# simplew4y/VeritasFi

Measured on AMD Instinct MI355X. Metric: queries/sec top-100 over 10Mx768 corpus, higher is better.
Workload: dtype f16

## Files before the change

veritasfi_amd/build.py:

```python
from __future__ import annotations

import os
import shutil
import subprocess
import sys

HERE = os.path.dirname(os.path.abspath(__file__))
CSRC = os.path.join(HERE, "csrc")
LIBDIR = os.path.join(HERE, "lib")
LIB = os.path.join(LIBDIR, os.environ.get("VF_BUILD_LIB", "libveritasfi_hip.so"))
SOURCES = ["vf_kernels.hip", "vf_api.hip", "vf_transformer.hip", "vf_sparse.hip"]
HEADERS = ["vf_internal.h", os.path.join("..", "..", "include", "veritasfi_hip.h"), "vf_ksplit_geom.h"]
ARCH = "gfx950"
FLAGS = ["-O3", "-std=c++17", "-fPIC", f"--offload-arch={ARCH}", "-Wall", "-Wno-unused-function"]
EXTRA = os.environ.get("VF_BUILD_FLAGS", "").split()


def _hipcc() -> str:
    for cand in (shutil.which("hipcc"), "/opt/rocm/bin/hipcc"):
        if cand and os.path.exists(cand):
            return cand
    raise RuntimeError("hipcc not found: the HIP library cannot be built (no fallback exists)")


def _stale(target: str, deps) -> bool:
    if not os.path.exists(target):
        return True
    t = os.path.getmtime(target)
    return any(os.path.exists(d) and os.path.getmtime(d) > t for d in deps)


KEPT_HOOKS = ("vf_debug_force_no_peer", "vf_debug_small_allocs")
TEST_LIB = os.path.join(LIBDIR, "libvf_test.so")


# ... 63 lines not shown
```

veritasfi_amd/csrc/vf_api.hip:

```cpp
#include "../../include/veritasfi_hip.h"
#include "vf_internal.h"

#include <fcntl.h>
#include <float.h>
#include <sys/stat.h>
#include <unistd.h>
#include <math.h>
#include <string.h>

#include <algorithm>
#include <atomic>
#include <mutex>
#include <string>
#include <vector>

using namespace vf;

static thread_local std::string g_err;

static int fail(int code, const std::string& msg) {
    g_err = msg;
    return code;
}
int vf::set_error(int code, const std::string& msg) { return fail(code, msg); }
// ... 181 lines not shown
            ix->rows_scan = ix->rows_orig;
            ix->owns_scan = false;
        } else {
            VF_HIP(hipMalloc((void**)&ix->rows_scan, (size_t)ix->n * ix->dp * scan_esz));
            ix->owns_scan = true;
            scan_out = ix->rows_scan;
        }
    }
    VF_HIP(launch_prep_rows(ix->rows_orig, dt, ix->n, ix->d, ix->dp, scan_out, ix->norm, ix->inv_scan, nullptr));
    VF_TRY(build_image(ix, ix->scan_image));
    if (ix->n > 0 && ix->n <= kSmallN) {
        VF_HIP(hipMalloc((void**)&ix->cn_cache, (size_t)ix->n * ix->d * sizeof(float)));
        VF_HIP(launch_normalize_rows(ix->rows_orig, dt, 0, ix->n, ix->d, ix->norm, ix->cn_cache, nullptr));
    }
    VF_HIP(hipDeviceSynchronize());
    return VF_OK;
}

constexpr int64_t kSplitMaxRows = 6'000'000;
constexpr int64_t kScan2rMinRows = 1'100'000;
static bool scan2r_auto_width(int dp, bool f8) { return f8 ? (dp == 768 || dp == 1024) : (dp == 768 || dp == 1024 || dp == 512 || dp == 384); }
static int64_t split_limit(const vf_index* ix) {
    const bool r_rows = ix->dtype != VF_DTYPE_FP8_E4M3 && ix->scan_impl != 4 && ix->scan_impl != 1 && ix->scan_impl != 3 && !ix->steal_opt &&
                        scan2r_auto_width(ix->dp, false) && scan2r_stage_cap(ix->dp, kMaxBatch, 0) >= 256;
    return r_rows ? INT64_MAX : kSplitMaxRows;
}
static int64_t resolved_aux(const vf_index* ix) {
    if (ix->aux_applied >= 0) return ix->aux_applied;
    int64_t a = ix->aux_cus >= 0 ? ix->aux_cus : (ix->n <= split_limit(ix) ? 32 : 0);
    if (a <= 0 || ix->n_cu < 64 || a * 2 > ix->n_cu) return 0;
    return a;
}
static bool resolved_overlap(const vf_index* ix) {
    return ix->overlap_scans >= 0 ? ix->overlap_scans != 0 : resolved_aux(ix) > 0;
}

constexpr int kImageMaxK = 128;
constexpr int64_t kImageMinRows = 4'000'000;
constexpr double kImageMaxRho = 1.0 / 64;
constexpr size_t kImageHeadroom = (size_t)8 << 30;
constexpr int kImageMfmaAuto = 1;
static bool image_eligible(const vf_index* ix) {
    return ix->shards.empty() && (ix->dtype == VF_DTYPE_F16 || ix->dtype == VF_DTYPE_F32) && ix->n >= kImageMinRows &&
           ix->n < (int64_t)0xFFFFFFFFll && ix->dp == 768 && scan2r_stage_cap(ix->dp, kMaxBatch, 2) >= 256;
}
static float* image_offsets(const vf_index* ix) { return ix->inv_img ? ix->inv_img + ix->n + 64 : nullptr; }
static void free_image(vf_index* ix) {
    if (ix->rows_img) (void)hipFree(ix->rows_img);
    if (ix->inv_img) (void)hipFree(ix->inv_img);
    ix->rows_img = nullptr; ix->inv_img = nullptr; ix->rho_max = ix->rho_mean = 0.0f;
}
static int build_image(vf_index* ix, int64_t mode) {
    if (mode == 0 || ix->rows_img || !image_eligible(ix)) return VF_OK;
    const size_t bytes = (size_t)ix->n * ix->dp, ibytes = 2 * ((size_t)ix->n + 64) * sizeof(float);
    if (mode == 1) {
        size_t free_b = 0, total_b = 0;
        if (hipMemGetInfo(&free_b, &total_b) != hipSuccess) { (void)hipGetLastError(); return VF_OK; }
        if (free_b < bytes + ibytes + kImageHeadroom) return VF_OK;
    }
    if (hipMalloc((void**)&ix->rows_img, bytes) != hipSuccess || hipMalloc((void**)&ix->inv_img, ibytes) != hipSuccess) {
        (void)hipGetLastError();
        free_image(ix);
        return mode == 2 ? fail(VF_ENOMEM, "scan_image = 2: the int8 row image does not fit in device memory") : VF_OK;
    }
    u32* d_rho = nullptr;
    VF_HIP(hipMalloc((void**)&d_rho, 2 * sizeof(u32)));
    VF_HIP(hipMemset(d_rho, 0, 2 * sizeof(u32)));
// ... 458 lines not shown
    *tau_band = (int)ceil(band * (kHistBins / 2)) + 1;
    *fine_band = (int)ceil(band * (kHistBins / 2) * 16) + 1;
}

extern "C" int vf_debug_image_bound(int32_t d, int32_t dtype, float rho_mean, float* eps, int32_t* tau_band, int32_t* fine_band) {
    if (!eps || !tau_band || !fine_band || d <= 0) return fail(VF_EINVAL, "vf_debug_image_bound: bad argument");
    int tb = 0, fb = 0;
    image_bound(d, dtype, rho_mean, eps, &tb, &fb);
    *tau_band = tb; *fine_band = fb;
    return VF_OK;
}

extern "C" int vf_debug_image_q8_bound(float rho_q, float eps_img, int32_t tau_band, int32_t fine_band, float* eps_q, int32_t* tau_band_q,
                                       int32_t* fine_band_q) {
    if (!eps_q || !tau_band_q || !fine_band_q) return fail(VF_EINVAL, "vf_debug_image_q8_bound: bad argument");
    const Q8Bound b = image_q8_bound(rho_q);
    *eps_q = image_q8_eps(eps_img, b.eps_add);
    *tau_band_q = tau_band + b.tau_bins; *fine_band_q = fine_band + b.fine_bins;
    return VF_OK;
}

static int image_planes(const vf_index* ix, int qt) {
    const int m = ix->image_mfma < 0 ? kImageMfmaAuto : (int)ix->image_mfma;
    return (m >= 1 && scan2r_stage_cap(ix->dp, qt, 2 + m) >= 256) ? m : 0;
}

static bool image_serves(const vf_index* ix, int k, int qt) {
    return ix->rows_img && k <= kImageMaxK && (ix->scan_impl == 2 || ix->scan_impl == 5) && !ix->steal_opt && ix->sample_impl != 0 &&
           scan2r_stage_cap(ix->dp, qt, 2) >= 256;
}

static FusedPlan make_plan(const vf_index* ix, int k, bool image = false) {
    FusedPlan p;
    p.image = image; p.tau_band = 0; p.fine_band = 0;
    int margin = ix->margin >= 0 ? (int)ix->margin : std::max(24, k / 4);
    const double u16 = 1.0 / 2048.0;
    const float eps_plan = (float)(u16 * (ix->dtype == VF_DTYPE_F32 ? 2.0 : 1.0) + sqrt((double)ix->d) * ldexp(1.0, -24) +
                                   2.0 * ix->d * ldexp(1.0, -24) + 1e-6);
    if (ix->margin < 0 && ksplit_width(ix)) {
        const double z = sqrt(2.0 * log(std::max(3.0, (double)ix->n / k)));
        margin = std::max(margin, (int)ceil(2.5 * eps_plan * k * z * sqrt((double)ix->d)));
    }
    p.kprime = ix->margin >= 0 ? k + margin : (k + margin + 31) / 32 * 32;
    p.kprime = std::min(p.kprime, 4096);
    int cap = kMaxCap;
    while (cap < 4 * p.kprime && cap < 16384) cap <<= 1;
    if (ix->cap_opt > 0) { cap = 1; while (cap < ix->cap_opt) cap <<= 1; cap = std::min(cap, 16384); }
    while (cap < 2 * p.kprime) cap <<= 1;
    p.cap = cap;
    const int64_t scan_cus = ix->n_cu - resolved_aux(ix);
    int64_t wgs = std::min<int64_t>(scan_cus, std::max<int64_t>(1, ix->n / 512));
    if (ix->waves_opt > 0) wgs = std::max<int64_t>(1, ix->waves_opt / (kScanThreads / 64));
// ... 206 lines not shown
            VF_TRY(s.qimg8.ensure((size_t)ix->dp * kMaxBatch * 2));
            VF_TRY(s.epsq.ensure(kMaxBatch * sizeof(float)));
            VF_TRY(s.qscale.ensure(kMaxBatch * sizeof(float)));
            VF_TRY(s.bandq.ensure(2 * kMaxBatch * sizeof(int)));
            VF_HIP(launch_prep_q8(qn_b, nb, ix->d, ix->dp, qt, s.image_i8, (signed char*)s.qimg8.p, s.qscale.as<float>(), s.epsq.as<float>(), s.bandq.as<int>(),
                                  p.eps, p.tau_band, p.fine_band, st));
            a.qimg = (const _Float16*)s.qimg8.p; a.q_scale = s.qscale.as<float>(); a.band_q = s.bandq.as<int>();
        }
        a.n = ix->n; a.dp = ix->dp; a.row_bytes = (long long)ix->dp * (ix->dtype == VF_DTYPE_FP8_E4M3 ? 1 : 2); a.total_waves = p.total_waves; a.samp = p.samp;
        if (p.image) { a.rows = (const char*)ix->rows_img; a.inv_scan = ix->inv_img; a.off_scan = image_offsets(ix); a.row_bytes = ix->dp; }
        a.s0 = s.s0.as<float>(); a.wg_base = s.wgbase.as<long long>(); a.cnt = s.cnt.as<u32>(); a.tau_bin = s.tau.as<int>(); a.hist = s.hist.as<u32>();
        a.cand = s.cand.as<u64>(); a.cap = p.cap; a.kprime = p.kprime; a.tau_band = p.tau_band;
        a.hist_coarse = s.hist_coarse.as<u32>(); a.stage_cap = ks ? scan_ksplit_stage_cap(ix->dp) : scan_stage_cap(ix->dp, qt);
        a.tile_cnt = ix->steal_opt ? s.tilecnt.as<u32>() : nullptr; a.scan_grid = p.grid;
        a.dbg = nullptr;
        if (ix->debug & 128) { VF_TRY(s.dbg.ensure((size_t)p.total_waves * ((ix->debug & 512) ? 72 : 4) * sizeof(u64))); a.dbg = s.dbg.as<u64>(); if (ix->debug & 512) VF_HIP(hipMemsetAsync(s.dbg.p, 0, s.dbg.bytes, st)); }
        a.refresh_every = (int)std::min<int64_t>(256, std::max<int64_t>(4, std::max<int64_t>(1, ix->refresh_every) * nb / kMaxBatch));
        while (a.refresh_every & (a.refresh_every - 1)) a.refresh_every &= a.refresh_every - 1;
        a.nq = nb; a.debug = (int)ix->debug;
        if (ix->n / p.total_waves < p.samp)
            VF_HIP(hipMemsetAsync(a.s0, 0xFF, (size_t)qt * p.total_waves * p.samp * sizeof(float), st));
        const bool f8rows = ix->dtype == VF_DTYPE_FP8_E4M3 || p.image;
        const bool r_f8_auto = f8rows && ix->scan_impl == 2 && ix->n > kScan2rMinRows && !ix->steal_opt && scan2r_auto_width(ix->dp, true);
        const bool sample_r = p.image || (ix->sample_impl != 0 && ix->scan_impl != 1 && scan2r_stage_cap(ix->dp, qt, f8rows) >= 256 &&
                              (ix->sample_impl == 1 || (!f8rows && s.scan_stream != s.stream && scan2r_auto_width(ix->dp, false)) || r_f8_auto));
        if (ks) {
            VF_HIP(launch_scan_ksplit(a, kModeSample, p.grid, st));
        } else if (sample_r) {
            const int64_t sg_r = ix->sample_grid > 0 ? ix->sample_grid : (s.scan_stream != s.stream ? resolved_aux(ix) : p.grid);
            ScanArgs as = a;
            as.stage_cap = 0;
            VF_HIP(launch_scan2r_sample(as, qt, (int)std::min<int64_t>(std::max<int64_t>(sg_r, 1), p.grid), p.image ? img_f8 : (int)f8rows, st));
        } else {
        const int64_t sg_opt = ix->sample_grid >= 0 ? ix->sample_grid : (s.scan_stream != s.stream ? 4 * resolved_aux(ix) : 0);
        const int sgrid = sg_opt > 0 ? (int)std::min<int64_t>(sg_opt, p.grid) : p.grid;
        VF_HIP(launch_scan(a, kModeSample, qt, sgrid, (int)ix->scan_g, ix->dtype == VF_DTYPE_FP8_E4M3, st));
        }
        VF_HIP(launch_sel0(a, qt, st));
        hipStream_t sst = s.scan_stream;
        if (sst != st) {
            VF_HIP(hipEventRecord(s.ev_pro, st));
            VF_HIP(hipStreamWaitEvent(sst, s.ev_pro, 0));
        }
        if (!resolved_overlap(ix))
            for (int o = 0; o < kSlots; ++o)
                if (o != slot_id && ix->slots[o].ev_scan) VF_HIP(hipStreamWaitEvent(sst, ix->slots[o].ev_scan, 0));
        if (s.timed && b0 == 0) {
// ... 2 lines not shown
                VF_HIP(hipEventRecord(ix->ev_span, sst));
                ix->span_started = true;
            }
            ix->span_slot[slot_id] = true;
            VF_HIP(hipEventRecord(s.ev_t[0], sst));
        }
        const int f8 = ix->dtype == VF_DTYPE_FP8_E4M3 ? 1 : 0;
        const int cap2 = ((ix->scan_impl == 3 || ((ix->scan_impl == 2 || ix->scan_impl == 4 || ix->scan_impl == 5) && !f8)) && !ix->steal_opt) ? scan2_stage_cap(ix->dp, qt, f8) : 0;
        const bool r_auto = ix->scan_impl == 2 && ix->n > kScan2rMinRows && scan2r_auto_width(ix->dp, f8 != 0) && (f8 || (s.scan_stream != s.stream && resolved_overlap(ix)));
#ifdef VF_EXPERIMENTS
        const bool dbg_r = f8 || !(ix->debug & (32 | 64));
#else
        const bool dbg_r = true;
#endif
        const int capr = ((ix->scan_impl == 5 || r_auto) && !ix->steal_opt && dbg_r) ? scan2r_stage_cap(ix->dp, qt, f8) : 0;
        if (ks) {
            VF_HIP(launch_scan_ksplit(a, kModeMain, p.grid, sst));
            s.scan_kernel = 6;
        } else if (p.image) {
            ScanArgs a2 = a;
            a2.stage_cap = scan2r_stage_cap(ix->dp, qt, img_f8);
            VF_HIP(launch_scan2r(a2, qt, p.grid, img_f8, sst));
            s.scan_kernel = 5;
        } else if (capr >= 256) {
            ScanArgs a2 = a;
            a2.stage_cap = capr;
            VF_HIP(launch_scan2r(a2, qt, p.grid, f8, sst));
            s.scan_kernel = 5;
        } else if (cap2 >= 256) {
            ScanArgs a2 = a;
            a2.stage_cap = cap2;
#ifdef VF_EXPERIMENTS
            if (ix->debug & 32) {
                const bool fresh = s.sib.bytes < 4096;
                VF_TRY(s.sib.ensure(4096));
                if (fresh) VF_HIP(hipMemsetAsync(s.sib.p, 0xFF, 4096, st));
                a2.sib = s.sib.as<u32>();
            }
#endif
            VF_HIP(launch_scan2(a2, qt, p.grid, f8, sst));
            s.scan_kernel = 2;
        } else {
            VF_HIP(launch_scan(a, kModeMain, qt, p.grid, (int)ix->scan_g, ix->dtype == VF_DTYPE_FP8_E4M3, sst));
            s.scan_kernel = 1;
        }
        VF_HIP(hipEventRecord(s.ev_scan, sst));
        if (s.timed && b0 == 0) {
// ... 729 lines not shown
```

veritasfi_amd/csrc/vf_internal.h:

```cpp
#pragma once
#include <hip/hip_runtime.h>
#include <math.h>
#include <stdint.h>

#include "../../include/veritasfi_hip.h"

#include <string>

#include "vf_ksplit_geom.h"

namespace vf {

int set_error(int code, const std::string& msg);

typedef unsigned long long u64;
typedef unsigned int u32;

struct DeviceGuard {
    int prev = -1;
    DeviceGuard() { if (hipGetDevice(&prev) != hipSuccess) prev = -1; }
    ~DeviceGuard() { if (prev >= 0) (void)hipSetDevice(prev); }
    DeviceGuard(const DeviceGuard&) = delete;
    DeviceGuard& operator=(const DeviceGuard&) = delete;
};

__device__ __forceinline__ u32 orderkey(float f) {
    f = f + 0.0f;
    const u32 b = __float_as_uint(f);
    return b ^ ((b >> 31) ? 0xFFFFFFFFu : 0x80000000u);
}
__device__ __forceinline__ float unorderkey(u32 k) {
    return __uint_as_float((k & 0x80000000u) ? (k ^ 0x80000000u) : ~k);
// ... 98 lines not shown
hipError_t launch_prep_rows(const void* rows, int dt , long long n, int d, int dp,
                            void* scan ,
                            float* norm, float* inv_scan, hipStream_t s);
hipError_t launch_prep_image(const void* rows, int dt, long long n, int d, int dp, const float* norm, unsigned char* img,
                             float* inv_img, float* off_img, u32* rho_max_bits, float* rho_sum, hipStream_t s);
hipError_t launch_prep_queries(const float* q, int nq, int d, int dp, int qn_tile ,
                               float* qn, _Float16* qimg, hipStream_t s);
hipError_t launch_normalize_rows(const void* rows, int dt , long long row0, long long nrows, int d,
                                 const float* norm, float* out, hipStream_t s);
hipError_t launch_normalize_rows_gather(const void* rows, int dt, const long long* sel , int nsel, int d,
                                        const float* norm, float* out, hipStream_t s);
hipError_t launch_dense_dot16(const float* qn, int nq, const float* cn, long long nrows, int d,
                              float* out, long long out_stride, hipStream_t s);
hipError_t launch_sort_rows(const float* scores, long long score_stride, int nq, int n, int k,
                            long long id_base, long long* out_ids, float* out_scores, int out_stride,
                            hipStream_t s);
hipError_t launch_scan(const ScanArgs& a, int mode, int qn_tile, int grid, int want_g ,
                       int rows_are_fp8, hipStream_t s);
hipError_t launch_debug_cvt_e4m3(const unsigned char* in, float* out, int count, hipStream_t s);
hipError_t launch_debug_mfma_i8(const signed char* A, const signed char* B, int* C, hipStream_t s);
hipError_t launch_scan2(const ScanArgs& a, int qn_tile, int grid, int rows_are_fp8, hipStream_t s);
size_t scan2_lds_bytes(int dp, int qn_tile, int stage_cap);
int scan2_stage_cap(int dp, int qn_tile, int rows_are_fp8);
size_t scan2r_lds_bytes(int dp, int qn_tile, int stage_cap, int f8);
int scan2r_stage_cap(int dp, int qn_tile, int f8);
hipError_t launch_scan2r(const ScanArgs& a, int qn_tile, int grid, int f8, hipStream_t s);
hipError_t launch_scan2r_sample(const ScanArgs& a, int qn_tile, int grid, int f8, hipStream_t s);
hipError_t launch_scan_ksplit(const ScanArgs& a, int mode, int grid, hipStream_t s);
size_t scan_ksplit_lds_bytes(int dp, int stage_cap);
int scan_ksplit_stage_cap(int dp);
hipError_t launch_scan_wide(const ScanArgs& a, int mode, int rows_are_fp8, hipStream_t s);
size_t scan_wide_lds_bytes(int stage_cap);
hipError_t launch_prep_wide8(const float* qn, int nq, int d, int dp, int qtot, unsigned char* img8, float* eps_q, hipStream_t s);
hipError_t launch_scan_wide8(const ScanArgs& a, int waves , hipStream_t s);
int scan_wide8_stage_cap(int waves);
int scan_wide8_occupancy(int waves, int stage_cap);
hipError_t launch_prep_q8(const float* qn, int nq, int d, int dp, int qn_tile, int planes , signed char* img8, float* q_scale, float* eps_q, int* band_q,
                          float eps_img, int tau_band, int fine_band, hipStream_t s);
hipError_t launch_sel0(const ScanArgs& a, int qn_tile, hipStream_t s);
hipError_t launch_final(FinalArgs a, int nq, hipStream_t s);
hipError_t launch_merge_topk(const long long* ids_parts, const float* score_parts, int nparts, int nq,
                             int k, long long* ids, float* scores, hipStream_t s);
hipError_t launch_merge_topk_packed(const void* parts, int nparts, int nq, int k, long long* ids, float* scores,
                                    hipStream_t s);
hipError_t launch_fuse_rank(const float* a, const float* b, int n, float* out, long long* order,
                            hipStream_t s);
// ... 7 lines not shown
```

veritasfi_amd/csrc/vf_kernels.hip:

```cpp
#include "vf_internal.h"

#include <float.h>
#include <algorithm>
#include <type_traits>

#include <mutex>

namespace vf {

typedef _Float16 h8 __attribute__((ext_vector_type(8)));
typedef _Float16 h4 __attribute__((ext_vector_type(4)));
typedef float f16v __attribute__((ext_vector_type(16)));
typedef int i4v __attribute__((ext_vector_type(4)));
typedef int i16v __attribute__((ext_vector_type(16)));
typedef int i8v __attribute__((ext_vector_type(8)));

__device__ __forceinline__ float group16_tree(float acc) {
    acc = acc + __shfl_down(acc, 8, 16);
    acc = acc + __shfl_down(acc, 4, 16);
    acc = acc + __shfl_down(acc, 2, 16);
    acc = acc + __shfl_down(acc, 1, 16);
    return acc;
}

// ... 727 lines not shown
                 __builtin_amdgcn_readlane((int)v, 32) | __builtin_amdgcn_readlane((int)v, 48));
}
__device__ __forceinline__ u32 wave_sum_u32(u32 v) {
    v += VF_DPP_ROR(v, 1);
    v += VF_DPP_ROR(v, 2);
    v += VF_DPP_ROR(v, 4);
    v += VF_DPP_ROR(v, 8);
    return (u32)(__builtin_amdgcn_readlane((int)v, 0) + __builtin_amdgcn_readlane((int)v, 16) +
                 __builtin_amdgcn_readlane((int)v, 32) + __builtin_amdgcn_readlane((int)v, 48));
}

template <int NT, int MODE>
__device__ __forceinline__ void epi_prefetch(EpiRegs<NT>& e, const ScanArgs& a, long long t0, int lane, bool sync_tau) {
    e.inv_lane = a.inv_scan[t0 + (lane & 31)];
    e.sync_tau = sync_tau;
    if (MODE == kModeMain && sync_tau) {
#pragma unroll
        for (int nt = 0; nt < NT; ++nt)
            e.tau_g[nt] = __hip_atomic_load(a.tau_bin + nt * kQueryTile + (lane & 31), __ATOMIC_RELAXED,
                                            __HIP_MEMORY_SCOPE_AGENT);
    }
}

template <int NT, int MODE, bool PUBLISH = true, bool INV_LDS = false, bool OFF = false>
__device__ __forceinline__ void tile_epilogue(const ScanArgs& a, const f16v (&acc)[NT], const EpiRegs<NT>& e,
                                              long long t0, long long hi, long long s0_slot, int lane, char* ctl) {
    const int r31 = lane & 31, h = lane >> 5;
    auto inv_of = [&](int reg) {
        const int r0 = (reg & 3) + 8 * (reg >> 2);
        const float lo_half = __builtin_bit_cast(float, __builtin_amdgcn_readlane(__builtin_bit_cast(int, e.inv_lane), r0));
        const float hi_half = __builtin_bit_cast(float, __builtin_amdgcn_readlane(__builtin_bit_cast(int, e.inv_lane), r0 + 4));
        return h ? hi_half : lo_half;
    };
    auto off_of = [&](int reg) {
        const int r0 = (reg & 3) + 8 * (reg >> 2);
        const float lo_half = __builtin_bit_cast(float, __builtin_amdgcn_readlane(__builtin_bit_cast(int, e.off_lane), r0));
        const float hi_half = __builtin_bit_cast(float, __builtin_amdgcn_readlane(__builtin_bit_cast(int, e.off_lane), r0 + 4));
        return h ? hi_half : lo_half;
    };
    if (MODE == kModeSample) {
        const long long s0_stride = (long long)a.total_waves * a.samp;
#pragma unroll
        for (int nt = 0; nt < NT; ++nt) {
            const int q = nt * kQueryTile + r31;
#pragma unroll
            for (int reg = 0; reg < 16; ++reg) {
                const int rr = (reg & 3) + 8 * (reg >> 2) + 4 * h;
                if constexpr (OFF) {
                    if (t0 + rr < hi) a.s0[(long long)q * s0_stride + s0_slot + rr] = acc[nt][reg] * inv_of(reg) + off_of(reg);
// ... 53 lines not shown
        }
        any |= bin_x(top) >= tb[nt];
    }
    if (__ballot(any) == 0ull) return;
    u32 mask = 0;
#pragma unroll
    for (int nt = 0; nt < NT; ++nt)
#pragma unroll
        for (int reg = 0; reg < 16; ++reg) mask |= (bin_x(m[nt * 16 + reg]) >= tb[nt]) ? (1u << (nt * 16 + reg)) : 0u;
    const unsigned long long hot = __ballot(mask != 0u);
    if (hot == 0ull) return;
    if (a.debug & 4) return;
    u32 umask = 0u, total = 0u;
    if (__popcll(hot) <= 8) {
        for (unsigned long long hb = hot; hb != 0ull; hb &= hb - 1ull) {
            const u32 m = (u32)__builtin_amdgcn_readlane((int)mask, __builtin_ctzll(hb));
            umask |= m;
            total += (u32)__popc(m);
        }
    } else {
        umask = wave_or_u32(mask);
        total = wave_sum_u32((u32)__popc(mask));
    }
    u32* stage_cnt = (u32*)ctl;
    uint4* stage_ent = (uint4*)(ctl + kCtlBytes);
    const u32 rs = 31u - (u32)__builtin_clz((u32)a.refresh_every | 1u);
    const u32 R = 1u << rs;
    u32 base = 0;
    if (lane == 0) base = atomicAdd(stage_cnt, total);
    base = (u32)__builtin_amdgcn_readfirstlane((int)base);
    const bool need = (base >> rs) != ((base + total) >> rs);
    if (a.debug & 8) return;
    u32 run = base;
    const u32 edge = (((base + total) >> rs) << rs) - 1u;
    int qq = 0;
    for (u32 um = umask; um != 0u; um &= um - 1u) {
        const int pair = __builtin_ctz(um);
        const int nt = pair >> 4, reg = pair & 15;
        const int q = nt * kQueryTile + r31;
        const bool mine = ((mask >> pair) & 1u) != 0u;
        const unsigned long long bal = __ballot(mine);
        if (mine) {
            const u32 slot = run + __builtin_amdgcn_mbcnt_hi((u32)(bal >> 32), __builtin_amdgcn_mbcnt_lo((u32)bal, 0u));
            const int rr = (reg & 3) + 8 * (reg >> 2) + 4 * h;
            const float sc = m[pair];
            const u32 bin = (u32)bin_of_x(bin_x(sc));
            const u32 key = orderkey(sc), row = (u32)(t0 + rr);
            if (slot < (u32)a.stage_cap) {
                stage_ent[slot] = make_uint4(row, key, (u32)q | (bin << 8), 1u);
            } else {
                const u32 gs = atomicAdd(a.cnt + q * kCntStride, 1u);
                if (gs < (u32)a.cap) a.cand[(long long)q * a.cap + gs] = ((u64)key << 32) | (u64)row;
                atomicAdd(a.hist + (long long)q * kHistBins + bin, 1u);
                atomicAdd(a.hist_coarse + q * 64 + (bin >> 5), 1u);
            }
        }
        const u32 nxt = run + (u32)__popcll(bal);
        if (run <= edge && edge < nxt) qq = nt * kQueryTile + ((__ffsll((long long)bal) - 1) & 31);
        run = nxt;
    }
    if (a.debug & 2) return;
    if constexpr (!PUBLISH) return;
    if (need) {
        const int nb = wave_tau_two_level(a.hist_coarse + qq * 64, a.hist + (long long)qq * kHistBins, a.kprime, lane) - (a.band_q ? a.band_q[qq] : a.tau_band);
        if (lane == 0 && nb > 0) {
            atomicMax(a.tau_bin + qq, nb);
            atomicMax(tau_lds + qq, nb);
        }
        for (u32 blk = base >> rs; blk < (base + total) >> rs; ++blk)
        for (u32 j = (u32)lane; j < R; j += 64u) {
            const u32 idx = (blk << rs) + j;
            if (idx >= (u32)a.stage_cap) break;
            const uint4 en = stage_ent[idx];
            if (en.w == 1u) {
                const u32 q = en.z & 0xFFu, bin = en.z >> 8;
                if (q < (u32)QN_of<NT>() && bin < (u32)kHistBins) {
                    atomicAdd(a.hist + (long long)q * kHistBins + bin, 1u);
                    atomicAdd(a.hist_coarse + q * 64 + (bin >> 5), 1u);
                }
            }
        }
    }
}

#define VF_ISSUE(BUF, ...)                                                        \
    do {                                                                          \
        if constexpr (F8 != 0) issue_loads_f8<G>(BUF, __VA_ARGS__);               \
        else issue_loads<G>(BUF, __VA_ARGS__);                                    \
    } while (0)
#define VF_COMPUTE(ACC, BUF, ...)                                                 \
    do {                                                                          \
        if constexpr (F8 != 0) compute_superstep_f8<NT, G>(ACC, BUF, __VA_ARGS__); \
        else compute_superstep<NT, G>(ACC, BUF, __VA_ARGS__);                      \
    } while (0)

// ... 638 lines not shown
        for (u32 i = tid; i < nst; i += kScan2Threads) {
            const uint4 e = ent[i];
            const u32 q = e.z & 0xFFu;
            if (e.w != 1u || q >= (u32)QN) continue;
            ent[i].w = 2u + atomicAdd(qcnt + q, 1u);
        }
        __syncthreads();
        if (tid < QN) {
            const u32 c = qcnt[tid];
            qbase[tid] = c ? atomicAdd(a.cnt + tid * kCntStride, c) : 0u;
        }
        __syncthreads();
        for (u32 i = tid; i < nst; i += kScan2Threads) {
            const uint4 e = ent[i];
            if (e.w < 2u) continue;
            const u32 q = e.z & 0xFFu;
            const u32 gs = qbase[q] + (e.w - 2u);
            if (gs < (u32)a.cap) a.cand[(long long)q * a.cap + gs] = ((u64)e.y << 32) | (u64)e.x;
        }
    }
    if (dbg) dbg[3] = wall_clock64();
}

struct Scan2rShape { int S, RB, RING; };
static Scan2rShape scan2r_shape(int dp, int f8) {
    if (!f8 && dp == 768) return {12, 6, 6};
    if (!f8 && dp == 1024) return {16, 6, 4};
    if (!f8 && dp == 512) return {8, 4, 6};
    if (!f8 && dp == 384) return {6, 3, 6};
    if (f8 == 3) return dp == 768 ? Scan2rShape{6, 6, 6} : Scan2rShape{0, 0, 0};
    if (f8 == 4) return dp == 768 ? Scan2rShape{6, 3, 6} : Scan2rShape{0, 0, 0};
    if (f8 && dp == 768) return {6, 3, 6};
    if (f8 && dp == 1024) return {8, 3, 4};
    return {0, 0, 0};
}

size_t scan2r_lds_bytes(int dp, int qn_tile, int stage_cap, int f8) {
    const Scan2rShape sh = scan2r_shape(dp, f8);
    const size_t seg_img = (size_t)(f8 ? 128 : 64) * qn_tile * 2;
    return (size_t)(sh.S - sh.RB) * seg_img + (size_t)kScan2Waves * (sh.RING * kSegBytes + kScratchBytes) + kCtlBytes + (size_t)stage_cap * 16;
}
int scan2r_stage_cap(int dp, int qn_tile, int f8) {
    if (scan2r_shape(dp, f8).S == 0) return 0;
    const size_t fixed = scan2r_lds_bytes(dp, qn_tile, 0, f8);
    if (fixed + 256 * 16 > 160 * 1024) return 0;
    const size_t area = std::min<size_t>(160 * 1024 - fixed, 32 * 1024);
    return (int)(area / 16);
}

template <int NT, int MODE, int F8 = 0, int S = 12, int RB = 6, int RING = 6, int AR = 1>
__global__ __launch_bounds__(kScan2Waves * 64) void k_scan2r(ScanArgs a) {
    const unsigned long long t_entry = (a.debug & 512) ? wall_clock64() : 0ull;
    const unsigned long long c_entry = (a.debug & 512) ? __builtin_amdgcn_s_memtime() : 0ull;
    extern __shared__ __attribute__((aligned(1024))) char smem[];
    constexpr int QN = NT * kQueryTile, THREADS = kScan2Waves * 64;
    constexpr bool I8 = F8 >= 3;
    constexpr int PLANES = F8 == 4 ? 2 : 1;
    constexpr int J = I8 ? 4 * PLANES : F8 ? 8 : 4;
    constexpr int SEGIMG = J * 2 * QN * 16;
    auto frag_off = [](int j) { return I8 ? (2 * (j & 3) * PLANES + (j >> 2)) * (QN * 16) : F8 ? ((j >> 2) * 8 + (j & 3)) * (QN * 16) : j * (QN * 16); };
    static_assert(F8 != 3 || RB == S, "the single int8 plane lives in registers whole: no LDS part");
    static_assert(S >= RING && RB <= S && RB <= 6, "ring fill and the spelled-out register segments");
    const int tid = threadIdx.x, lane = tid & 63, wid = tid >> 6;
    const int r31 = lane & 31, h = lane >> 5;
    const long long grid = (MODE == kModeSample && a.scan_grid > 0) ? a.scan_grid : gridDim.x;
    const long long swg = (long long)a.samp * (kScanThreads / 64);
    const int tps = (int)((swg + kRowTile - 1) / kRowTile);
    long long lo = 0, hi = 0;
    int ntiles;
    if (MODE == kModeSample) {
        const long long mine = (grid - (long long)blockIdx.x + gridDim.x - 1) / gridDim.x;
        ntiles = (int)(mine > 0 ? mine : 0) * tps;
    } else {
        const long long Ra = a.n * blockIdx.x / grid, Rb = a.n * (blockIdx.x + 1) / grid;
// ... 13 lines not shown
            t0 = lo + (long long)tile * kRowTile; thi = hi; sbase = 0;
        }
    };
    h8 breg[RB][J][NT];
    {
        const char* qb = (const char*)a.qimg + ((long long)((I8 ? PLANES : 4) * h) * QN + r31) * 16;
#pragma unroll
        for (int sg = 0; sg < RB; ++sg)
#pragma unroll
            for (int j = 0; j < J; ++j)
#pragma unroll
                for (int nt = 0; nt < NT; ++nt)
                    breg[sg][j][nt] = *(const h8*)(qb + (long long)sg * SEGIMG + frag_off(j) + nt * (kQueryTile * 16));
    }
    float sq[NT];
#pragma unroll
    for (int nt = 0; nt < NT; ++nt) sq[nt] = I8 ? a.q_scale[nt * kQueryTile + r31] : 1.0f;
    char* ring = smem + (size_t)wid * (RING * kSegBytes);
    char* img = smem + kScan2Waves * RING * kSegBytes;
    constexpr size_t kImgBytes = (size_t)(S - RB) * SEGIMG;
    char* scratch = img + kImgBytes + (size_t)wid * kScratchBytes;
    char* ctl = img + kImgBytes + kScan2Waves * kScratchBytes;
    u32* next_tile = (u32*)(ctl + 4);
    const unsigned ring_l = (unsigned)__builtin_amdgcn_readfirstlane((int)lds_addr(ring)), scratch_l = (unsigned)__builtin_amdgcn_readfirstlane((int)lds_addr(scratch));
    const int drow = lane >> 3;
    struct TileSrc { unsigned long long ua; unsigned v[4]; };
    auto src_of = [&](int tile) -> TileSrc {
        long long t0_, thi_, sb_;
        tile_rows(tile, t0_, thi_, sb_);
        TileSrc ts;
        const long long last_row = thi_ - 1 > 0 ? thi_ - 1 : 0;
        long long base_row = t0_ > 0 ? t0_ : 0;
        base_row = base_row < last_row ? base_row : last_row;
        ts.ua = (unsigned long long)(a.rows + base_row * a.row_bytes);
        ts.ua = ((unsigned long long)(unsigned)__builtin_amdgcn_readfirstlane((int)(ts.ua >> 32)) << 32) | (unsigned)__builtin_amdgcn_readfirstlane((int)ts.ua);
#pragma unroll
        for (int m = 0; m < 4; ++m) {
            const int row = 8 * m + drow;
            long long r = t0_ + row;
            r = r < last_row ? r : last_row;
            r = r > base_row ? r : base_row;
            ts.v[m] = (unsigned)((r - base_row) * a.row_bytes) + ((((lane & 7) ^ ((row >> 1) & 7))) << 4);
        }
        return ts;
    };
    auto first_row = [&](int tile) {
// ... 16 lines not shown
    if (active) {
        src_cur = src_of(cur_tile);
        issue_epi(first_row(cur_tile), MODE == kModeMain, 0);
#pragma unroll
        for (int sg = 0; sg < RING; ++sg) issue_seg(src_cur, sg, sg);
    }
    typedef unsigned int u4r __attribute__((ext_vector_type(4)));
    {
        const char* srcq = (const char*)a.qimg + (long long)RB * SEGIMG;
        constexpr int nkb = (int)(kImgBytes >> 10);
        const unsigned img_l = (unsigned)__builtin_amdgcn_readfirstlane((int)lds_addr(img));
        const int wu = __builtin_amdgcn_readfirstlane(wid);
        for (int c = wu; c < nkb; c += kScan2Waves) dma16(srcq + ((long long)c << 10) + (lane << 4), img_l + ((unsigned)c << 10));
        __builtin_amdgcn_s_waitcnt(0x0F70);
        if constexpr (AR) {
#pragma unroll
            for (int sg = 0; sg < RB; ++sg)
#pragma unroll
                for (int j = 0; j < J; ++j)
#pragma unroll
                    for (int nt = 0; nt < NT; ++nt) asm volatile("" : "+a"(breg[sg][j][nt]));
        }
        uint4* z = (uint4*)ctl;
        const int nz = kCtlBytes / 16 + (MODE == kModeMain ? a.stage_cap : 0);
        for (int i = tid; i < nz; i += THREADS) z[i] = make_uint4(0u, (i == 0) ? (u32)kScan2Waves : 0u, 0u, 0u);
    }
    __syncthreads();
    if (MODE == kModeMain) {
        if (tid < QN) ((int*)(ctl + 16))[tid] = a.tau_bin[tid];
        __syncthreads();
    }

    const char* lds_lane = img + (((I8 ? PLANES : 4) * h) * QN + r31) * 16;
    const int asw = (r31 >> 1) & 7;
    const char* a_lane = ring + r31 * 128;
    const int dbg_rec = (a.debug & 512) ? 72 : 4;
    unsigned long long* dbg = (MODE == kModeMain && (a.debug & 128) && a.dbg && lane == 0) ? a.dbg + ((long long)blockIdx.x * kScan2Waves + wid) * dbg_rec : nullptr;
    if (dbg) dbg[0] = wall_clock64();
    if (dbg && dbg_rec > 4) {
        dbg[68] = t_entry;
        unsigned hw_id, xcc_id;
        asm volatile("s_getreg_b32 %0, hwreg(HW_REG_HW_ID)\n\ts_getreg_b32 %1, hwreg(HW_REG_XCC_ID)" : "=s"(hw_id), "=s"(xcc_id));
        dbg[70] = ((unsigned long long)xcc_id << 32) | hw_id;
    }
#ifdef VF_EXPERIMENTS
    const bool prof = (a.debug & 4096) != 0;
    unsigned long long pc_wait = 0, pc_use = 0, pc_fill = 0, pc_head = 0, pc_epi = 0, pc_n = 0, pt0 = 0, pt1 = 0;
    auto cyc = [&]() { unsigned long long t; asm volatile("s_memtime %0\n\ts_waitcnt lgkmcnt(0)" : "=s"(t) :: "memory"); return t; };
// ... 155 lines not shown
            }
            VF_PC(pt0 = cyc())
            const char* sc = scratch + (tiles_done & 1) * 512;
            EpiRegs<NT> epi;
            epi.inv_lane = *(const float*)(sc + 256 + r31 * 4);
            epi.inv_lds = sc + 256;
            if constexpr (F8 >= 2) epi.off_lane = *(const float*)(sc + 384 + r31 * 4);
            if constexpr (I8) {
#pragma unroll
                for (int nt = 0; nt < NT; ++nt)
#pragma unroll
                    for (int e = 0; e < 16; ++e) {
                        float v = (float)acci[0][nt][e];
                        if constexpr (PLANES == 2) { v = v * 254.0f + (float)acci[1][nt][e]; acci[1][nt][e] = 0; }
                        acc[nt][e] = v * sq[nt];
                        acci[0][nt][e] = 0;
                    }
            }
            epi.sync_tau = sync_now;
            if (sync_now) {
#pragma unroll
                for (int nt = 0; nt < NT; ++nt) epi.tau_g[nt] = *(const int*)(sc + (nt * kQueryTile + r31) * 4);
            }
            tile_epilogue<NT, MODE, true, true, F8 >= 2>(a, acc, epi, t0, t_hi, t_s0, lane, ctl);
#pragma unroll
            for (int nt = 0; nt < NT; ++nt)
#pragma unroll
                for (int e = 0; e < 16; ++e) acc[nt][e] = 0.0f;
            VF_PC(pt1 = cyc(); pc_epi += pt1 - pt0)
            ++tiles_done;
            if (!more) break;
            cur_tile = nxt;
            src_cur = src_nxt;
        }
    }
    if (dbg && dbg_rec > 4) dbg[69] = (unsigned long long)tiles_done;
    asm volatile("s_waitcnt vmcnt(0)" ::: "memory");
    if (MODE == kModeSample) return;
    if (lane == 0) atomicAdd((u32*)(ctl + 8), 1u);
    if (dbg) dbg[1] = wall_clock64();
    __syncthreads();
    if (dbg) dbg[2] = wall_clock64();
    {
        const u32 staged = *(const u32*)ctl;
        const u32 nst = staged < (u32)a.stage_cap ? staged : (u32)a.stage_cap;
        uint4* ent = (uint4*)(ctl + kCtlBytes);
        u32* qcnt = (u32*)(kImgBytes ? img : smem);
        u32* qbase = qcnt + QN;
        if (tid < QN) qcnt[tid] = 0u;
        __syncthreads();
        for (u32 i = tid; i < nst; i += THREADS) {
            const uint4 e = ent[i];
            const u32 q = e.z & 0xFFu;
            if (e.w != 1u || q >= (u32)QN) continue;
            ent[i].w = 2u + atomicAdd(qcnt + q, 1u);
        }
        __syncthreads();
        if (tid < QN) {
            const u32 c = qcnt[tid];
            qbase[tid] = c ? atomicAdd(a.cnt + tid * kCntStride, c) : 0u;
        }
        __syncthreads();
        for (u32 i = tid; i < nst; i += THREADS) {
            const uint4 e = ent[i];
            if (e.w < 2u) continue;
            const u32 q = e.z & 0xFFu;
            const u32 gs = qbase[q] + (e.w - 2u);
            if (gs < (u32)a.cap) a.cand[(long long)q * a.cap + gs] = ((u64)e.y << 32) | (u64)e.x;
        }
    }
    if (dbg && dbg_rec > 4) dbg[71] = __builtin_amdgcn_s_memtime() - c_entry;
#ifdef VF_EXPERIMENTS
    if (dbg && dbg_rec > 4 && prof) { dbg[4] = pc_wait; dbg[5] = pc_use; dbg[6] = pc_fill; dbg[7] = pc_head; dbg[8] = pc_epi; dbg[9] = pc_n; }
#endif
#undef VF_PC
    if (dbg) dbg[3] = wall_clock64();
}

constexpr int kWideQ = 256, kWideNT = kWideQ / kQueryTile, kWideKC = 64, kWideRows = 256;
#ifndef VF_WIDE_THREADS
#define VF_WIDE_THREADS 512
#endif
constexpr int kWideThreads = VF_WIDE_THREADS, kWideWaves = kWideThreads / 64, kWideM = kWideRows / kWideWaves / kRowTile;
constexpr int kWideBuf = (kWideKC / 8) * kWideQ * 16;
constexpr int kWideCtl = 16 + 3 * kWideQ * 4;
constexpr int kSampWaves = kScanThreads / 64;

template <int F8> struct WideStage { uint4 w[kWideM][4]; };
template <int F8> __device__ __forceinline__ constexpr int wide_dc() { return F8 ? 2 : 1; }

template <int F8>
__device__ __forceinline__ void wide_issue_a(WideStage<F8>& st, const char* rows, long long row_bytes, const long long (&row)[kWideM],
                                             int unit, int h) {
#pragma unroll
    for (int m = 0; m < kWideM; ++m) {
        if constexpr (F8 != 0) {
// ... 1557 lines not shown
```

Baseline: 48580.

## Replace block-shared candidate stage with per-wave LDS stages drained incrementally

Each wave in k_scan2r now owns a private LDS staging region for candidate entries instead of a block-wide stage guarded by an LDS atomic counter. When the region fills, the wave drains it to global candidates via a wave-local prefix count. The end-of-kernel block-wide drain with its __syncthreads barriers is replaced by a final per-wave drain. The kernel also gets a waves_per_eu(1,1) attribute, and the LDS geometry moves into a shared header. Each wave's stage is smaller, so there may be more mid-scan drains, and publish granularity changes.

```diff
diff --git a/veritasfi_amd/build.py b/veritasfi_amd/build.py
--- a/veritasfi_amd/build.py
+++ b/veritasfi_amd/build.py
@@ -10,7 +10,7 @@
 LIBDIR = os.path.join(HERE, "lib")
 LIB = os.path.join(LIBDIR, os.environ.get("VF_BUILD_LIB", "libveritasfi_hip.so"))
 SOURCES = ["vf_kernels.hip", "vf_api.hip", "vf_transformer.hip", "vf_sparse.hip"]
-HEADERS = ["vf_internal.h", os.path.join("..", "..", "include", "veritasfi_hip.h"), "vf_ksplit_geom.h"]
+HEADERS = ["vf_internal.h", os.path.join("..", "..", "include", "veritasfi_hip.h"), "vf_ksplit_geom.h", "vf_stage_geom.h"]
 ARCH = "gfx950"
 FLAGS = ["-O3", "-std=c++17", "-fPIC", f"--offload-arch={ARCH}", "-Wall", "-Wno-unused-function"]
 EXTRA = os.environ.get("VF_BUILD_FLAGS", "").split()
diff --git a/veritasfi_amd/csrc/vf_api.hip b/veritasfi_amd/csrc/vf_api.hip
--- a/veritasfi_amd/csrc/vf_api.hip
+++ b/veritasfi_amd/csrc/vf_api.hip
@@ -227,7 +227,7 @@
 static bool scan2r_auto_width(int dp, bool f8) { return f8 ? (dp == 768 || dp == 1024) : (dp == 768 || dp == 1024 || dp == 512 || dp == 384); }
 static int64_t split_limit(const vf_index* ix) {
     const bool r_rows = ix->dtype != VF_DTYPE_FP8_E4M3 && ix->scan_impl != 4 && ix->scan_impl != 1 && ix->scan_impl != 3 && !ix->steal_opt &&
-                        scan2r_auto_width(ix->dp, false) && scan2r_stage_cap(ix->dp, kMaxBatch, 0) >= 256;
+                        scan2r_auto_width(ix->dp, false) && scan2r_stage_cap(ix->dp, kMaxBatch, 0) >= kScan2rMinStage;
     return r_rows ? INT64_MAX : kSplitMaxRows;
 }
 static int64_t resolved_aux(const vf_index* ix) {
@@ -247,7 +247,7 @@
 constexpr int kImageMfmaAuto = 1;
 static bool image_eligible(const vf_index* ix) {
     return ix->shards.empty() && (ix->dtype == VF_DTYPE_F16 || ix->dtype == VF_DTYPE_F32) && ix->n >= kImageMinRows &&
-           ix->n < (int64_t)0xFFFFFFFFll && ix->dp == 768 && scan2r_stage_cap(ix->dp, kMaxBatch, 2) >= 256;
+           ix->n < (int64_t)0xFFFFFFFFll && ix->dp == 768 && scan2r_stage_cap(ix->dp, kMaxBatch, 2) >= kScan2rMinStage;
 }
 static float* image_offsets(const vf_index* ix) { return ix->inv_img ? ix->inv_img + ix->n + 64 : nullptr; }
 static void free_image(vf_index* ix) {
@@ -752,12 +752,12 @@
 
 static int image_planes(const vf_index* ix, int qt) {
     const int m = ix->image_mfma < 0 ? kImageMfmaAuto : (int)ix->image_mfma;
-    return (m >= 1 && scan2r_stage_cap(ix->dp, qt, 2 + m) >= 256) ? m : 0;
+    return (m >= 1 && scan2r_stage_cap(ix->dp, qt, 2 + m) >= kScan2rMinStage) ? m : 0;
 }
 
 static bool image_serves(const vf_index* ix, int k, int qt) {
     return ix->rows_img && k <= kImageMaxK && (ix->scan_impl == 2 || ix->scan_impl == 5) && !ix->steal_opt && ix->sample_impl != 0 &&
-           scan2r_stage_cap(ix->dp, qt, 2) >= 256;
+           scan2r_stage_cap(ix->dp, qt, 2) >= kScan2rMinStage;
 }
 
 static FusedPlan make_plan(const vf_index* ix, int k, bool image = false) {
@@ -1010,7 +1010,7 @@
             VF_HIP(hipMemsetAsync(a.s0, 0xFF, (size_t)qt * p.total_waves * p.samp * sizeof(float), st));
         const bool f8rows = ix->dtype == VF_DTYPE_FP8_E4M3 || p.image;
         const bool r_f8_auto = f8rows && ix->scan_impl == 2 && ix->n > kScan2rMinRows && !ix->steal_opt && scan2r_auto_width(ix->dp, true);
-        const bool sample_r = p.image || (ix->sample_impl != 0 && ix->scan_impl != 1 && scan2r_stage_cap(ix->dp, qt, f8rows) >= 256 &&
+        const bool sample_r = p.image || (ix->sample_impl != 0 && ix->scan_impl != 1 && scan2r_stage_cap(ix->dp, qt, f8rows) >= kScan2rMinStage &&
                               (ix->sample_impl == 1 || (!f8rows && s.scan_stream != s.stream && scan2r_auto_width(ix->dp, false)) || r_f8_auto));
         if (ks) {
             VF_HIP(launch_scan_ksplit(a, kModeSample, p.grid, st));
@@ -1059,7 +1059,7 @@
             a2.stage_cap = scan2r_stage_cap(ix->dp, qt, img_f8);
             VF_HIP(launch_scan2r(a2, qt, p.grid, img_f8, sst));
             s.scan_kernel = 5;
-        } else if (capr >= 256) {
+        } else if (capr >= kScan2rMinStage) {
             ScanArgs a2 = a;
             a2.stage_cap = capr;
             VF_HIP(launch_scan2r(a2, qt, p.grid, f8, sst));
diff --git a/veritasfi_amd/csrc/vf_internal.h b/veritasfi_amd/csrc/vf_internal.h
--- a/veritasfi_amd/csrc/vf_internal.h
+++ b/veritasfi_amd/csrc/vf_internal.h
@@ -8,6 +8,7 @@
 #include <string>
 
 #include "vf_ksplit_geom.h"
+#include "vf_stage_geom.h"
 
 namespace vf {
 
@@ -152,6 +153,7 @@
 hipError_t launch_scan2(const ScanArgs& a, int qn_tile, int grid, int rows_are_fp8, hipStream_t s);
 size_t scan2_lds_bytes(int dp, int qn_tile, int stage_cap);
 int scan2_stage_cap(int dp, int qn_tile, int rows_are_fp8);
+constexpr int kScan2rMinStage = vf::kStageMinEntries;
 size_t scan2r_lds_bytes(int dp, int qn_tile, int stage_cap, int f8);
 int scan2r_stage_cap(int dp, int qn_tile, int f8);
 hipError_t launch_scan2r(const ScanArgs& a, int qn_tile, int grid, int f8, hipStream_t s);
diff --git a/veritasfi_amd/csrc/vf_kernels.hip b/veritasfi_amd/csrc/vf_kernels.hip
--- a/veritasfi_amd/csrc/vf_kernels.hip
+++ b/veritasfi_amd/csrc/vf_kernels.hip
@@ -773,9 +773,54 @@
     }
 }
 
-template <int NT, int MODE, bool PUBLISH = true, bool INV_LDS = false, bool OFF = false>
+struct WaveStage {
+    u32* qcnt = nullptr;
+    __device__ __forceinline__ uint4* ent() const { return (uint4*)(qcnt + vf::kStageQueries); }
+    u32 cap = 0, n = 0;
+    u32 since = 0;
+#ifdef VF_EXPERIMENTS
+    u32 n_global = 0, n_drains = 0;
+#endif
+};
+
+template <int QN>
+__device__ __forceinline__ void wave_stage_drain(const ScanArgs& a, WaveStage& ws, int lane, u32 pub_shift) {
+    const u32 nst = ws.n < ws.cap ? ws.n : ws.cap;
+    uint4* ent = ws.ent();
+    ws.qcnt[lane] = 0u;
+    __builtin_amdgcn_wave_barrier();
+    for (u32 i = (u32)lane; i < nst; i += 64u) ent[i].w = atomicAdd(ws.qcnt + (ent[i].z & 0xFFu), 1u);
+    __builtin_amdgcn_wave_barrier();
+    const u32 c = ws.qcnt[lane];
+    u32 gbase = 0u;
+    if (c != 0u) gbase = atomicAdd(a.cnt + lane * kCntStride, c);
+    for (u32 i0 = 0u; i0 < nst; i0 += 64u) {
+        const u32 i = i0 + (u32)lane;
+        const bool valid = i < nst;
+        const uint4 e = ent[valid ? i : 0u];
+        const u32 q = e.z & 0xFFu;
+        const u32 gs = (u32)__shfl((int)gbase, (int)q) + e.w;
+        if (valid && q < (u32)QN && gs < (u32)a.cap) a.cand[(long long)q * a.cap + gs] = ((u64)e.y << 32) | (u64)e.x;
+    }
+    if (!(a.debug & 2)) {
+        for (u32 i = ((ws.n >> pub_shift) << pub_shift) + (u32)lane; i < nst; i += 64u) {
+            const u32 z = ent[i].z, q = z & 0xFFu, bin = z >> 8;
+            if (q < (u32)QN && bin < (u32)kHistBins) {
+                atomicAdd(a.hist + (long long)q * kHistBins + bin, 1u);
+                atomicAdd(a.hist_coarse + q * 64 + (bin >> 5), 1u);
+            }
+        }
+    }
+    asm volatile("s_waitcnt vmcnt(0)" ::: "memory");
+    ws.n = 0u;
+#ifdef VF_EXPERIMENTS
+    ++ws.n_drains;
+#endif
+}
+
+template <int NT, int MODE, bool PUBLISH = true, bool INV_LDS = false, bool OFF = false, bool WSTAGE = false>
 __device__ __forceinline__ void tile_epilogue(const ScanArgs& a, const f16v (&acc)[NT], const EpiRegs<NT>& e,
-                                              long long t0, long long hi, long long s0_slot, int lane, char* ctl) {
+                                              long long t0, long long hi, long long s0_slot, int lane, char* ctl, WaveStage* ws = nullptr) {
     const int r31 = lane & 31, h = lane >> 5;
     auto inv_of = [&](int reg) {
         const int r0 = (reg & 3) + 8 * (reg >> 2);
@@ -875,17 +920,36 @@
         umask = wave_or_u32(mask);
         total = wave_sum_u32((u32)__popc(mask));
     }
-    u32* stage_cnt = (u32*)ctl;
+    const u32 rs = 31u - (u32)__builtin_clz((u32)a.refresh_every | 1u);
+    const u32 ps = WSTAGE ? (rs > 2u ? rs - 2u : 0u) : rs;
+    const u32 R = 1u << ps;
+    u32 stage_cap = (u32)a.stage_cap;
     uint4* stage_ent = (uint4*)(ctl + kCtlBytes);
-    const u32 rs = 31u - (u32)__builtin_clz((u32)a.refresh_every | 1u);
-    const u32 R = 1u << rs;
     u32 base = 0;
-    if (lane == 0) base = atomicAdd(stage_cnt, total);
-    base = (u32)__builtin_amdgcn_readfirstlane((int)base);
-    const bool need = (base >> rs) != ((base + total) >> rs);
-    if (a.debug & 8) return;
+    if constexpr (WSTAGE) {
+        if (ws->n != 0u && ws->n + total > ws->cap) wave_stage_drain<QN_of<NT>()>(a, *ws, lane, ps);
+        base = ws->n;
+        ws->n = base + total;
+        stage_cap = ws->cap;
+        stage_ent = ws->ent();
+    } else {
+        if (lane == 0) base = atomicAdd((u32*)ctl, total);
+        base = (u32)__builtin_amdgcn_readfirstlane((int)base);
+    }
+    bool need = (base >> rs) != ((base + total) >> rs);
+    u32 edge = (((base + total) >> rs) << rs) - 1u;
+    if constexpr (WSTAGE) {
+        const u32 cnt = ws->since + total, rem = cnt & ((1u << ps) - 1u);
+        need = (cnt >> ps) != 0u;
+        edge = base + total - rem - 1u;
+        ws->since = rem;
+    }
+    const bool pub = (base >> ps) != ((base + total) >> ps);
+    if (a.debug & 8) {
+        if constexpr (WSTAGE) ws->n = base;
+        return;
+    }
     u32 run = base;
-    const u32 edge = (((base + total) >> rs) << rs) - 1u;
     int qq = 0;
     for (u32 um = umask; um != 0u; um &= um - 1u) {
         const int pair = __builtin_ctz(um);
@@ -899,7 +963,7 @@
             const float sc = m[pair];
             const u32 bin = (u32)bin_of_x(bin_x(sc));
             const u32 key = orderkey(sc), row = (u32)(t0 + rr);
-            if (slot < (u32)a.stage_cap) {
+            if (slot < stage_cap) {
                 stage_ent[slot] = make_uint4(row, key, (u32)q | (bin << 8), 1u);
             } else {
                 const u32 gs = atomicAdd(a.cnt + q * kCntStride, 1u);
@@ -908,6 +972,9 @@
                 atomicAdd(a.hist_coarse + q * 64 + (bin >> 5), 1u);
             }
         }
+#ifdef VF_EXPERIMENTS
+        if constexpr (WSTAGE) ws->n_global += (u32)__popcll(__ballot(mine && run + __builtin_amdgcn_mbcnt_hi((u32)(bal >> 32), __builtin_amdgcn_mbcnt_lo((u32)bal, 0u)) >= stage_cap));
+#endif
         const u32 nxt = run + (u32)__popcll(bal);
         if (run <= edge && edge < nxt) qq = nt * kQueryTile + ((__ffsll((long long)bal) - 1) & 31);
         run = nxt;
@@ -920,10 +987,12 @@
             atomicMax(a.tau_bin + qq, nb);
             atomicMax(tau_lds + qq, nb);
         }
-        for (u32 blk = base >> rs; blk < (base + total) >> rs; ++blk)
+    }
+    if (pub) {
+        for (u32 blk = base >> ps; blk < (base + total) >> ps; ++blk)
         for (u32 j = (u32)lane; j < R; j += 64u) {
-            const u32 idx = (blk << rs) + j;
-            if (idx >= (u32)a.stage_cap) break;
+            const u32 idx = (blk << ps) + j;
+            if (idx >= stage_cap) break;
             const uint4 en = stage_ent[idx];
             if (en.w == 1u) {
                 const u32 q = en.z & 0xFFu, bin = en.z >> 8;
@@ -1608,34 +1677,20 @@
     if (dbg) dbg[3] = wall_clock64();
 }
 
-struct Scan2rShape { int S, RB, RING; };
-static Scan2rShape scan2r_shape(int dp, int f8) {
-    if (!f8 && dp == 768) return {12, 6, 6};
-    if (!f8 && dp == 1024) return {16, 6, 4};
-    if (!f8 && dp == 512) return {8, 4, 6};
-    if (!f8 && dp == 384) return {6, 3, 6};
-    if (f8 == 3) return dp == 768 ? Scan2rShape{6, 6, 6} : Scan2rShape{0, 0, 0};
-    if (f8 == 4) return dp == 768 ? Scan2rShape{6, 3, 6} : Scan2rShape{0, 0, 0};
-    if (f8 && dp == 768) return {6, 3, 6};
-    if (f8 && dp == 1024) return {8, 3, 4};
-    return {0, 0, 0};
-}
+using vf::Scan2rShape;
+using vf::scan2r_shape;
+static_assert(vf::kStageWaves == kScan2Waves && vf::kStageSegBytes == kSegBytes && vf::kStageScratchBytes == kScratchBytes && vf::kStageCtlBytes == kCtlBytes,
+              "vf_stage_geom.h states k_scan2r's carve-up");
 
 size_t scan2r_lds_bytes(int dp, int qn_tile, int stage_cap, int f8) {
-    const Scan2rShape sh = scan2r_shape(dp, f8);
-    const size_t seg_img = (size_t)(f8 ? 128 : 64) * qn_tile * 2;
-    return (size_t)(sh.S - sh.RB) * seg_img + (size_t)kScan2Waves * (sh.RING * kSegBytes + kScratchBytes) + kCtlBytes + (size_t)stage_cap * 16;
+    return (size_t)vf::scan2r_total_bytes(dp, qn_tile, f8, kScan2Waves, stage_cap);
 }
 int scan2r_stage_cap(int dp, int qn_tile, int f8) {
-    if (scan2r_shape(dp, f8).S == 0) return 0;
-    const size_t fixed = scan2r_lds_bytes(dp, qn_tile, 0, f8);
-    if (fixed + 256 * 16 > 160 * 1024) return 0;
-    const size_t area = std::min<size_t>(160 * 1024 - fixed, 32 * 1024);
-    return (int)(area / 16);
+    return vf::scan2r_wave_cap(dp, qn_tile, f8, kScan2Waves);
 }
 
 template <int NT, int MODE, int F8 = 0, int S = 12, int RB = 6, int RING = 6, int AR = 1>
-__global__ __launch_bounds__(kScan2Waves * 64) void k_scan2r(ScanArgs a) {
+__global__ __launch_bounds__(kScan2Waves * 64) __attribute__((amdgpu_waves_per_eu(1, 1))) void k_scan2r(ScanArgs a) {
     const unsigned long long t_entry = (a.debug & 512) ? wall_clock64() : 0ull;
     const unsigned long long c_entry = (a.debug & 512) ? __builtin_amdgcn_s_memtime() : 0ull;
     extern __shared__ __attribute__((aligned(1024))) char smem[];
@@ -1695,6 +1750,12 @@
     char* scratch = img + kImgBytes + (size_t)wid * kScratchBytes;
     char* ctl = img + kImgBytes + kScan2Waves * kScratchBytes;
     u32* next_tile = (u32*)(ctl + 4);
+    WaveStage ws;
+    if (MODE == kModeMain) {
+        char* region = ctl + kCtlBytes + (size_t)wid * (size_t)vf::scan2r_region_bytes(a.stage_cap);
+        ws.qcnt = (u32*)region;
+        ws.cap = (u32)__builtin_amdgcn_readfirstlane(a.stage_cap);
+    }
     const unsigned ring_l = (unsigned)__builtin_amdgcn_readfirstlane((int)lds_addr(ring)), scratch_l = (unsigned)__builtin_amdgcn_readfirstlane((int)lds_addr(scratch));
     const int drow = lane >> 3;
     struct TileSrc { unsigned long long ua; unsigned v[4]; };
@@ -1757,8 +1818,7 @@
                     for (int nt = 0; nt < NT; ++nt) asm volatile("" : "+a"(breg[sg][j][nt]));
         }
         uint4* z = (uint4*)ctl;
-        const int nz = kCtlBytes / 16 + (MODE == kModeMain ? a.stage_cap : 0);
-        for (int i = tid; i < nz; i += THREADS) z[i] = make_uint4(0u, (i == 0) ? (u32)kScan2Waves : 0u, 0u, 0u);
+        for (int i = tid; i < kCtlBytes / 16; i += THREADS) z[i] = make_uint4(0u, (i == 0) ? (u32)kScan2Waves : 0u, 0u, 0u);
     }
     __syncthreads();
     if (MODE == kModeMain) {
@@ -1960,7 +2020,7 @@
 #pragma unroll
                 for (int nt = 0; nt < NT; ++nt) epi.tau_g[nt] = *(const int*)(sc + (nt * kQueryTile + r31) * 4);
             }
-            tile_epilogue<NT, MODE, true, true, F8 >= 2>(a, acc, epi, t0, t_hi, t_s0, lane, ctl);
+            tile_epilogue<NT, MODE, true, true, F8 >= 2, MODE == kModeMain>(a, acc, epi, t0, t_hi, t_s0, lane, ctl, &ws);
 #pragma unroll
             for (int nt = 0; nt < NT; ++nt)
 #pragma unroll
@@ -1975,41 +2035,17 @@
     if (dbg && dbg_rec > 4) dbg[69] = (unsigned long long)tiles_done;
     asm volatile("s_waitcnt vmcnt(0)" ::: "memory");
     if (MODE == kModeSample) return;
-    if (lane == 0) atomicAdd((u32*)(ctl + 8), 1u);
-    if (dbg) dbg[1] = wall_clock64();
-    __syncthreads();
-    if (dbg) dbg[2] = wall_clock64();
-    {
-        const u32 staged = *(const u32*)ctl;
-        const u32 nst = staged < (u32)a.stage_cap ? staged : (u32)a.stage_cap;
-        uint4* ent = (uint4*)(ctl + kCtlBytes);
-        u32* qcnt = (u32*)(kImgBytes ? img : smem);
-        u32* qbase = qcnt + QN;
-        if (tid < QN) qcnt[tid] = 0u;
-        __syncthreads();
-        for (u32 i = tid; i < nst; i += THREADS) {
-            const uint4 e = ent[i];
-            const u32 q = e.z & 0xFFu;
-            if (e.w != 1u || q >= (u32)QN) continue;
-            ent[i].w = 2u + atomicAdd(qcnt + q, 1u);
-        }
-        __syncthreads();
-        if (tid < QN) {
-            const u32 c = qcnt[tid];
-            qbase[tid] = c ? atomicAdd(a.cnt + tid * kCntStride, c) : 0u;
-        }
-        __syncthreads();
-        for (u32 i = tid; i < nst; i += THREADS) {
-            const uint4 e = ent[i];
-            if (e.w < 2u) continue;
-            const u32 q = e.z & 0xFFu;
-            const u32 gs = qbase[q] + (e.w - 2u);
-            if (gs < (u32)a.cap) a.cand[(long long)q * a.cap + gs] = ((u64)e.y << 32) | (u64)e.x;
-        }
+    if (dbg) dbg[1] = dbg[2] = wall_clock64();
+    if (ws.n != 0u) {
+        const u32 rs_ = 31u - (u32)__builtin_clz((u32)a.refresh_every | 1u);
+        wave_stage_drain<QN>(a, ws, lane, rs_ > 2u ? rs_ - 2u : 0u);
+#ifdef VF_EXPERIMENTS
+        --ws.n_drains;
+#endif
     }
     if (dbg && dbg_rec > 4) dbg[71] = __builtin_amdgcn_s_memtime() - c_entry;
 #ifdef VF_EXPERIMENTS
-    if (dbg && dbg_rec > 4 && prof) { dbg[4] = pc_wait; dbg[5] = pc_use; dbg[6] = pc_fill; dbg[7] = pc_head; dbg[8] = pc_epi; dbg[9] = pc_n; }
+    if (dbg && dbg_rec > 4 && prof) { dbg[4] = pc_wait; dbg[5] = pc_use; dbg[6] = pc_fill; dbg[7] = pc_head; dbg[8] = pc_epi; dbg[9] = pc_n; dbg[10] = ws.n_global; dbg[11] = ws.n_drains; }
 #endif
 #undef VF_PC
     if (dbg) dbg[3] = wall_clock64();
diff --git a/veritasfi_amd/csrc/vf_stage_geom.h b/veritasfi_amd/csrc/vf_stage_geom.h
--- /dev/null
+++ b/veritasfi_amd/csrc/vf_stage_geom.h
@@ -0,0 +1,54 @@
+#pragma once
+
+#if defined(__HIPCC__)
+#define VF_SG_HD __host__ __device__ __forceinline__
+#else
+#define VF_SG_HD inline
+#endif
+
+namespace vf {
+
+constexpr int kStageLdsBytes = 160 * 1024;
+constexpr int kStageWaves = 4;
+constexpr int kStageSegBytes = 4096;
+constexpr int kStageScratchBytes = 1024;
+constexpr int kStageCtlBytes = 272;
+constexpr int kStageEntryBytes = 16;
+constexpr int kStageQueries = 64;
+constexpr int kStageHeadBytes = kStageQueries * 4;
+constexpr int kStageMinEntries = 64;
+
+struct Scan2rShape { int S, RB, RING; };
+VF_SG_HD Scan2rShape scan2r_shape(int dp, int f8) {
+    if (!f8 && dp == 768) return {12, 6, 6};
+    if (!f8 && dp == 1024) return {16, 6, 4};
+    if (!f8 && dp == 512) return {8, 4, 6};
+    if (!f8 && dp == 384) return {6, 3, 6};
+    if (f8 == 3) return dp == 768 ? Scan2rShape{6, 6, 6} : Scan2rShape{0, 0, 0};
+    if (f8 == 4) return dp == 768 ? Scan2rShape{6, 3, 6} : Scan2rShape{0, 0, 0};
+    if (f8 && dp == 768) return {6, 3, 6};
+    if (f8 && dp == 1024) return {8, 3, 4};
+    return {0, 0, 0};
+}
+VF_SG_HD long long scan2r_fixed_bytes(int dp, int qn_tile, int f8, int waves) {
+    const Scan2rShape sh = scan2r_shape(dp, f8);
+    const long long seg_img = (long long)(f8 ? 128 : 64) * qn_tile * 2;
+    return (long long)(sh.S - sh.RB) * seg_img + (long long)waves * (sh.RING * kStageSegBytes + kStageScratchBytes) + kStageCtlBytes;
+}
+VF_SG_HD int scan2r_wave_cap(int dp, int qn_tile, int f8, int waves) {
+    if (scan2r_shape(dp, f8).S == 0 || waves < 1) return 0;
+    const long long left = (long long)kStageLdsBytes - scan2r_fixed_bytes(dp, qn_tile, f8, waves);
+    if (left <= 0) return 0;
+    const long long share = left / waves / kStageEntryBytes * kStageEntryBytes;
+    const long long cap = (share - kStageHeadBytes) / kStageEntryBytes;
+    return cap >= kStageMinEntries ? (int)cap : 0;
+}
+VF_SG_HD long long scan2r_region_bytes(int cap) { return (long long)kStageHeadBytes + (long long)cap * kStageEntryBytes; }
+VF_SG_HD long long scan2r_region_off(int dp, int qn_tile, int f8, int waves, int cap, int w) {
+    return scan2r_fixed_bytes(dp, qn_tile, f8, waves) + (long long)w * scan2r_region_bytes(cap);
+}
+VF_SG_HD long long scan2r_total_bytes(int dp, int qn_tile, int f8, int waves, int cap) {
+    return scan2r_fixed_bytes(dp, qn_tile, f8, waves) + (cap > 0 ? (long long)waves * scan2r_region_bytes(cap) : 0);
+}
+
+}
```

Result: slower. 40310 (-17.0%).
